# yuki-koyama/sequential-line-search

Hardware: AMD Instinct MI355X
Metric: GP-fit+acq-max step time (ms) and candidate-evals/sec at N=8192 D=64 (higher is better)
Workload: dtype f64

## Files before the change

### sequential-line-search_amd/csrc/capi.hip

```cpp
#include <cstddef>
#include <cstring>
#include <algorithm>
#include <cmath>
#include <cstdlib>
#include <cstring>
#include <atomic>
#include <map>
#include <memory>
#include <condition_variable>
#include <mutex>
#include <shared_mutex>

#include "common.hpp"
#include "kernels.hpp"
#include "lbfgs_driver.hpp"

using namespace slsk;


namespace slsk {
static thread_local char g_err[512] = "";
void set_error(const char* fmt, ...) {
    va_list ap;
    va_start(ap, fmt);
// ... 322 lines not shown
    if (launches) *launches = it == ctx->prof.end() ? 0 : it->second.launches;
    return SLS_OK;
}

static void h2d(sls_ctx* c, double* dst, const double* src, size_t n) {
    SLS_HIP(hipMemcpyAsync(dst, src, n * sizeof(double), hipMemcpyHostToDevice, c->stream));
}
static void d2h(sls_ctx* c, double* dst, const double* src, size_t n) {
    SLS_HIP(hipMemcpyAsync(dst, src, n * sizeof(double), hipMemcpyDeviceToHost, c->stream));
}
static void sync(sls_ctx* c) { SLS_HIP(hipStreamSynchronize(c->stream)); }
static const size_t IO_STAGE_MAX = (size_t)4 << 20;

static void check_theta(const double* theta, int D) {
    SLS_REQUIRE(theta != nullptr, "theta is NULL");
    SLS_REQUIRE(theta[0] > 0.0, "theta[0] (signal variance) must be positive");
    for (int d = 0; d < D; ++d) SLS_REQUIRE(theta[1 + d] > 0.0, "length scale %d must be positive", d);
}

static void d2h_matrix(sls_ctx* c, double* dst, const double* src, int N, int Np) {
    SLS_HIP(hipMemcpy2DAsync(dst, (size_t)N * 8, src, (size_t)Np * 8, (size_t)N * 8, N, hipMemcpyDeviceToHost, c->stream));
}
static void h2d_matrix(sls_ctx* c, double* dst, const double* src, int N, int Np) {
    SLS_HIP(hipMemcpy2DAsync(dst, (size_t)Np * 8, src, (size_t)N * 8, (size_t)N * 8, N, hipMemcpyHostToDevice, c->stream));
}

struct sls_gp {
    sls_ctx* ctx = nullptr;
    int D = 0, N = 0, Np = 0, Dp = 0, Dcols = 0, kernel = 0;
    double a = 0, b = 0;
    std::vector<double> theta, Xh, yh;
    std::vector<double> il_h, ypad_h;
    bool host_stale = false;
    DBuf X, y, inv_ell, XT, XaT, nx, L, Linv, Kinv, U, alpha, tvec, mu_data, scal, gemv_part, idx_buf;
    const double* linv_clean_p = nullptr;
    int linv_clean_np = 0;
    long* d_idx = nullptr;
    HostBuf sum;
    int best_index = 0;
    double mu_best = 0, logdet = 0;
    DBuf Ks, Cs, P, Vs, parts, Gs, Gm, Gpart, XsT, ns, raw, outv;
    int ws_chunk = 0;
    DBuf pair_mu, pair_sg, pair_dmu, pair_dsg;
    LbfgsWs lb;
    DBuf eubo_Ks, eubo_Cs, eubo_XsT, eubo_ns, eubo_parts, eubo_Gs, eubo_Gm, eubo_Kd;
    int eubo_chunk = 0, eubo_np = 0;
    HostBuf eubo_best;
    int sigma_mode = 0;
    long generation = 0;
    long stat_issued = 0, stat_cap = 0;
    int stat_rounds = 0, stat_live_end = 0;
    HostBuf zc;
    HostBuf io;
    double* io_stage(size_t doubles) {
        if (io.host && doubles * 8 > io.bytes) (void)hipStreamSynchronize(ctx->stream);
        io.ensure(ctx, doubles * 8, false);
        return io.host;
    }
    std::shared_mutex state_mtx;
};

static bool gp_fit_small_ok(const sls_gp* g) {
    if (g->N > NLL_SMALL_MAX_N || g->Np != 128 || g->D > 128) return false;
    return tune_on(TUNE_FIT_SMALL);
}

static std::atomic<long> g_gp_generation{0};
static void gp_fit_device(sls_gp* g) {
    g->generation = ++g_gp_generation;
    sls_ctx* c = g->ctx;
    const int N = g->N, Np = g->Np, D = g->D;
    if (gp_fit_small_ok(g)) {
        GpFitSmallArgs f;
        f.X = g->X.p; f.y = g->y.p; f.inv_ell = g->inv_ell.p;
        f.D = D; f.N = N; f.Dcols = g->Dcols; f.a = g->a; f.b = g->b;
        f.XT = g->XT.p; f.nx = g->nx.p; f.XaT = g->XaT.p; f.L = g->L.p; f.Linv = g->Linv.p; f.U = g->U.p; f.Kinv = g->Kinv.p;
        f.alpha = g->alpha.p; f.mu_data = g->mu_data.p; f.scal = g->scal.p; f.d_idx = g->d_idx; f.info = c->d_info;
        f.summary = g->sum.dev;
        f.x_lds = tune_on(TUNE_SMALL_XLDS) ? 1 : 0;
        SLS_HIP(hipMemsetAsync(c->d_info, 0, 64, c->stream));
        ProfScope ps(c, "fit_small");
        launch_gp_fit_small(c->stream, g->kernel, f);
        return;
    }
    KernelSpec ks{g->kernel, g->a};
    {
        ProfScope ps(c, "gram");
        launch_prep_points(c->stream, g->X.p, D, N, g->inv_ell.p, g->XT.p, Np, Np, g->Dcols, g->nx.p);
        launch_gram_sym(c->stream, g->XT.p, Np, g->Dp, g->nx.p, Np, N, ks, g->b, g->L.p, true);
    }
    SLS_HIP(hipMemsetAsync(c->d_info, 0, 64, c->stream));
    if (g->linv_clean_p != g->Linv.p || g->linv_clean_np != Np) {
        launch_fill(c->stream, g->Linv.p, (long)Np * Np, 0.0);
        g->linv_clean_p = g->Linv.p;
        g->linv_clean_np = Np;
    }
    c->potrf_tick_rearm();
    int* df_sync = c->potrf_df_sync(Np);
    if (potri_fused_applies(Np, df_sync != nullptr)) {
        ProfScope ps(c, "potri");
        if (!launch_potri(c->stream, g->L.p, Np, g->Linv.p, g->U.p, g->Kinv.p, c->d_info, df_sync))
            ps.rename("potrf+trtri+lauum");
    } else {
        {
            ProfScope ps(c, "potrf");
            launch_potrf(c->stream, g->L.p, Np, g->Linv.p, c->d_info, 0, df_sync);
        }
        {
            ProfScope ps(c, "trtri");
            launch_trtri(c->stream, g->L.p, Np, g->Linv.p, g->Kinv.p, g->U.p);
        }
        {
            ProfScope ps(c, "lauum");
            launch_lauum(c->stream, g->U.p, Np, g->Kinv.p);
        }
    }
    launch_gemv_n(c->stream, g->Linv.p, Np, g->y.p, g->tvec.p, g->gemv_part.p, true);
    launch_gemv_t(c->stream, g->Linv.p, Np, g->tvec.p, g->alpha.p, true);
    launch_scale_rows(c->stream, g->XT.p, g->alpha.p, g->XaT.p, Np, Np, g->Dcols);
    if (g->sigma_mode == 1) launch_transpose_full(c->stream, g->Linv.p, g->U.p, Np);
    launch_fit_summary(c->stream, g->y.p, g->alpha.p, g->b, N, g->mu_data.p, g->L.p, Np, c->d_info, g->scal.p, g->d_idx, g->sum.dev);
}

static void gp_fetch_summary(sls_gp* g, int attempt = 0) {
    sls_ctx* c = g->ctx;
    sync(c);
    const double* sm = g->sum.host;
    const int info[2] = {(int)sm[3], (int)sm[4]};
    if (potrf_gave_up(c, info[1], attempt)) {
        gp_fit_device(g);
        gp_fetch_summary(g, 1);
        return;
    }
    if (info[0] != 0) {
        set_error("Cholesky failed: K_y is not positive definite (pivot %d)", info[0] - 1);
        throw HipFail{SLS_ERR_NOT_SPD};
    }
    g->best_index = (int)sm[2];
    g->mu_best = sm[0];
    g->logdet = sm[1];
}
static void gp_setup(sls_gp* g) {
    sls_ctx* ctx = g->ctx;
    const int D = g->D, N = (int)g->yh.size();
    g->N = N;
    g->Np = round_up(N, 128); g->Dp = round_up(D, 16); g->Dcols = round_up(D, 128);
    const size_t Np = g->Np;
    g->X.ensure((size_t)D * N); g->y.ensure(Np); g->inv_ell.ensure(g->Dcols);
    g->XT.ensure(Np * g->Dcols); g->XaT.ensure(Np * g->Dcols); g->nx.ensure(Np);
    g->L.ensure(Np * Np); g->Linv.ensure(Np * Np); g->Kinv.ensure(Np * Np); g->U.ensure(Np * Np);
    g->alpha.ensure(Np); g->tvec.ensure(Np); g->mu_data.ensure(Np); g->scal.ensure(8);
    g->gemv_part.ensure((Np / 128) * Np);
    g->ws_chunk = 0;
    g->idx_buf.ensure(8);
    g->d_idx = reinterpret_cast<long*>(g->idx_buf.p);
    g->sum.ensure(ctx, (size_t)(16 + D) * 8, true);
    g->il_h.assign(g->Dcols, 0.0);
    g->ypad_h.assign(Np, 0.0);
    for (int d = 0; d < D; ++d) g->il_h[d] = 1.0 / g->theta[1 + d];
    std::copy(g->yh.begin(), g->yh.end(), g->ypad_h.begin());
    h2d(ctx, g->X.p, g->Xh.data(), (size_t)D * N);
    h2d(ctx, g->y.p, g->ypad_h.data(), Np);
    h2d(ctx, g->inv_ell.p, g->il_h.data(), g->Dcols);
    gp_fit_device(g);
    gp_fetch_summary(g);
}

extern "C" int sls_gp_create(sls_ctx* ctx, const double* X, int D, int N, const double* y, const double* theta, double b,
                             int kernel, sls_gp** out) {
    SLS_TRY
    CtxCall call_(ctx);
    SLS_REQUIRE(ctx && out, "sls_gp_create: NULL argument");
    SLS_REQUIRE(D >= 1 && N >= 1, "sls_gp_create: need D >= 1 and N >= 1 (got D=%d N=%d)", D, N);
    SLS_REQUIRE(X && y, "sls_gp_create: X / y is NULL");
    SLS_REQUIRE(kernel == SLS_KERNEL_ARD_SQUARED_EXPONENTIAL || kernel == SLS_KERNEL_ARD_MATERN52, "unknown kernel %d", kernel);
    SLS_REQUIRE(b >= 0.0, "noise level must be >= 0");
    check_theta(theta, D);
    SLS_HIP(hipSetDevice(ctx->device));
    std::unique_ptr<sls_gp> g(new sls_gp());
    g->ctx = ctx; g->D = D; g->kernel = kernel; g->a = theta[0]; g->b = b;
    g->theta.assign(theta, theta + D + 1);
    g->Xh.assign(X, X + (size_t)D * N);
// ... 192 lines not shown
            ProfScope ps(c, "cross_gram");
            if (point_major) launch_prep_points(c->stream, xr + (size_t)s0 * D, D, sc, g->inv_ell.p, g->XsT.p, ldk, Sp, g->Dcols, g->ns.p);
            else launch_prep_cands(c->stream, xr + s0, ldr, D, sc, g->inv_ell.p, g->XsT.p, ldk, Sp, g->Dcols, g->ns.p);
            launch_cross_gram(c->stream, g->XsT.p, ldk, g->ns.p, Sp, g->XT.p, Np, g->nx.p, Np, N, g->Dp, ks, g->alpha.p, g->Ks.p, Cs,
                              ldk, mu_part, ca_part);
        }
        int split_first = 0x7fffffff;
        const bool solve_grad = g->sigma_mode == 1 && (want_grad || !tri_predict());
        {
            ProfScope ps(c, want_grad ? "acq_gemm" : "var_gemm");
            if (solve_grad) {
                g->Vs.ensure((size_t)chunk_max * Np);
                launch_gemm_plain(c->stream, g->Ks.p, ldk, false, g->Linv.p, Np, false, g->Vs.p, ldk, Sp / 128, Np / 128, Np, 1.0, 0.0);
                split_first = launch_acq_gemm(c->stream, g->Vs.p, Cs, ldk, Sp, g->U.p, Np, g->P.p, kw_part, cw_part, c->d_info + 32);
            } else if (want_grad || !tri_predict())
                split_first = launch_acq_gemm(c->stream, g->Ks.p, Cs, ldk, Sp, g->Kinv.p, Np, g->P.p, kw_part, cw_part, c->d_info + 32);
            else
                launch_var_gemm(c->stream, g->Ks.p, ldk, Sp, g->Linv.p, Np, kw_part, cw_part);
        }
        double* kw_solve = nullptr;
        if (solve_grad) {
            kw_solve = cw_part + (size_t)2 * nbt * ldk;
            ProfScope ps(c, "var_gemm");
            launch_var_gemm(c->stream, g->Ks.p, ldk, Sp, g->Linv.p, Np, kw_solve, kw_solve + (size_t)2 * nbt * ldk);
        }
        if (want_grad) {
            ProfScope ps(c, "grad_gemm");
            double* part = nullptr;
            if (D <= 64 && grad_gemm_wants_split(Sp)) {
                g->Gpart.ensure((size_t)8 * Sp * 64);
                part = g->Gpart.p;
            }
            launch_grad_gemm(c->stream, g->P.p, Cs, ldk, Sp, g->XT.p, g->XaT.p, Np, Np, D <= 64 ? -g->Dcols : g->Dcols, g->Gs.p, g->Gm.p,
                             part);
        }
        {
            ProfScope ps(c, "finalize");
            FinalizeArgs f;
            f.S = sc; f.D = D; f.nbt = nbt; f.ldk = ldk; f.ntm = Sp / 128; f.split_first = split_first;
            f.mu_part = mu_part; f.ca_part = ca_part; f.kw_part = kw_part; f.cw_part = cw_part;
            f.kw_solve_part = kw_solve;
            f.Gs = g->Gs.p; f.Gm = g->Gm.p; f.XsT = g->XsT.p; f.inv_ell = g->inv_ell.p;
            f.a = g->a; f.mu_best = g->mu_best; f.ucb_h = o.ucb_h; f.acq = o.acq;
            f.ldo = o.ldo;
            f.mu = o.mu ? o.mu + s0 : nullptr;
            f.sigma = o.sigma ? o.sigma + s0 : nullptr;
            f.dmu = o.dmu ? o.dmu + s0 : nullptr;
            f.dsigma = o.dsigma ? o.dsigma + s0 : nullptr;
            f.val = o.val ? o.val + s0 : nullptr;
            f.grad = o.grad ? o.grad + s0 : nullptr;
            launch_finalize(c->stream, f);
        }
    }
}

constexpr int WAVE_PATH_MAX_POINTS = 4096;
static bool wave_path_dims(const sls_gp* g) { return tune_on(TUNE_WAVE_PATH) && g->D <= WAVE_PATH_MAX_D; }
static bool wave_path_applies(const sls_gp* g, int count) {
    return wave_path_dims(g) && g->Np <= WAVE_PATH_MAX_NP && count <= WAVE_PATH_MAX_POINTS;
}
static void wave_model_args(const sls_gp* g, WaveArgs& w) {
    w.D = g->D; w.N = g->N; w.Np = g->Np;
    w.matern = g->kernel == SLS_KERNEL_ARD_MATERN52;
    w.a = g->a; w.mu_best = g->mu_best;
    w.XT = g->XT.p; w.inv_ell = g->inv_ell.p; w.Kinv = g->Kinv.p; w.alpha = g->alpha.p;
    w.solve_sigma = g->sigma_mode == 1; w.Linv = g->Linv.p; w.U = g->U.p;
    w.useful = nullptr;
// ... 578 lines not shown
        }
        double* kw_solve = solve ? cw_part[0] + (size_t)2 * nbt * ldk : nullptr;
        for (int o = 0; o < 2; ++o) {
            ProfScope ps(c, "cross_gram");
            launch_prep_cands(c->stream, xr + (size_t)o * D * ldr + s0, ldr, D, sc, g->inv_ell.p, XsT[o], ldk, Sp, g->Dcols, ns[o]);
            launch_cross_gram(c->stream, XsT[o], ldk, ns[o], Sp, g->XT.p, Np, g->nx.p, Np, N, g->Dp, ks, g->alpha.p, Ks[o], Cs[o], ldk,
                              mu_part[o], ca_part[o]);
        }
        {
            ProfScope ps(c, "eubo");
            launch_pair_diff(c->stream, Ks[0], Ks[1], ldk, Np, g->eubo_Kd.p);
        }
        if (solve) {
            {
                ProfScope ps(c, "acq_gemm");
                launch_gemm_plain(c->stream, g->eubo_Kd.p, ldk, false, g->Linv.p, Np, false, g->Vs.p, ldk, Sp / 128, Np / 128, Np, 1.0, 0.0);
            }
            ProfScope ps(c, "var_gemm");
            launch_var_gemm(c->stream, g->eubo_Kd.p, ldk, Sp, g->Linv.p, Np, kw_solve, kw_solve + (size_t)2 * nbt * ldk);
        }
        int split_first = 0x7fffffff;
        for (int o = 0; o < 2; ++o) {
            {
                ProfScope ps(c, "acq_gemm");
                split_first = launch_acq_gemm(c->stream, solve ? g->Vs.p : g->eubo_Kd.p, Cs[o], ldk, Sp, solve ? g->U.p : g->Kinv.p, Np,
                                              g->P.p, kw_part[o], cw_part[o], c->d_info + 32);
            }
            ProfScope ps(c, "grad_gemm");
            double* part = nullptr;
            if (D <= 64 && grad_gemm_wants_split(Sp)) {
                g->Gpart.ensure((size_t)8 * Sp * 64);
                part = g->Gpart.p;
            }
            launch_grad_gemm(c->stream, g->P.p, Cs[o], ldk, Sp, g->XT.p, g->XaT.p, Np, Np, D <= 64 ? -g->Dcols : g->Dcols, Gs[o], Gm[o], part);
        }
        {
            ProfScope ps(c, "eubo");
            EuboFinalizeArgs f;
            f.S = sc; f.D = D; f.nbt = nbt; f.ntm = Sp / 128; f.split_first = split_first; f.kernel = g->kernel; f.ldk = ldk;
            for (int o = 0; o < 2; ++o) {
                f.mu_part[o] = mu_part[o]; f.ca_part[o] = ca_part[o]; f.cw_part[o] = cw_part[o];
                f.Gs[o] = Gs[o]; f.Gm[o] = Gm[o]; f.XsT[o] = XsT[o];
            }
            f.kw_part = kw_part[0]; f.kw_solve_part = kw_solve; f.inv_ell = g->inv_ell.p; f.a = g->a;
            f.ldo = ldo;
            f.val = val ? val + s0 : nullptr;
            f.grad = grad ? grad + s0 : nullptr;
            launch_eubo_finalize(c->stream, f);
        }
    }
}

extern "C" int sls_eubo_eval(sls_gp* g, const double* pairs, int M, double* val, double* grad) {
    SLS_TRY
    CtxCall call_(g);
    SLS_REQUIRE(g != nullptr, "sls_eubo_eval: gp is NULL");
    SLS_REQUIRE(pairs != nullptr, "sls_eubo_eval: pairs is NULL");
    SLS_REQUIRE(M >= 0, "sls_eubo_eval: M = %d", M);
    if (M == 0) return SLS_OK;
    std::shared_lock<std::shared_mutex> state_(g->state_mtx);
    sls_ctx* c = g->ctx;
    const int Mp = round_up(M, 128), D2 = 2 * g->D;
    std::vector<double> t((size_t)Mp * D2, 0.5);
    for (int m = 0; m < M; ++m)
        for (int r = 0; r < D2; ++r) t[(size_t)m + (size_t)r * Mp] = pairs[r + (size_t)m * D2];
    g->raw.ensure((size_t)Mp * D2);
    h2d(c, g->raw.p, t.data(), (size_t)Mp * D2);
// ... 201 lines not shown
    }
    g->Xh.insert(g->Xh.end(), x, x + D);
    g->yh.push_back(y_new);
    if (N % 128 == 0) {
        gp_setup(g);
        return SLS_OK;
    }
    upload_candidates(g, x, 1, g->raw, 128);
    ensure_eval_ws(g, 128);
    g->outv.ensure(4 * (size_t)Np + 8);
    double* kvec = g->outv.p;
    double* uvec = kvec + Np;
    double* lvec = uvec + Np;
    double* tmp = lvec + Np;
    double* scal = tmp + Np;
    KernelSpec ks{g->kernel, g->a};
    launch_prep_cands(c->stream, g->raw.p, 128, D, 1, g->inv_ell.p, g->XsT.p, 128, 128, g->Dcols, g->ns.p);
    double* Cs = (g->kernel == SLS_KERNEL_ARD_MATERN52) ? g->Cs.p : g->Ks.p;
    launch_cross_gram(c->stream, g->XsT.p, 128, g->ns.p, 128, g->XT.p, Np, g->nx.p, Np, N, g->Dp, ks, nullptr, g->Ks.p, Cs, 128,
                      nullptr, nullptr);
    SLS_HIP(hipMemcpy2DAsync(kvec, 8, g->Ks.p, 128 * 8, 8, Np, hipMemcpyDeviceToDevice, c->stream));
    launch_gemv_n(c->stream, g->Kinv.p, Np, kvec, uvec, g->gemv_part.p);
    launch_gemv_n(c->stream, g->Linv.p, Np, kvec, lvec, g->gemv_part.p, true);
    launch_append_dots(c->stream, kvec, uvec, lvec, g->y.p, N, scal);
    const double kappa = g->a + g->b;
    launch_append_update(c->stream, g->Kinv.p, g->L.p, g->Linv.p, g->alpha.p, Np, N, uvec, lvec, scal, kappa, y_new);
    SLS_HIP(hipMemcpyAsync(g->y.p + N, &g->yh[N], 8, hipMemcpyHostToDevice, c->stream));
    g->X.ensure((size_t)D * (N + 1));
    SLS_HIP(hipMemcpyAsync(g->X.p, g->Xh.data(), (size_t)D * (N + 1) * 8, hipMemcpyHostToDevice, c->stream));
    g->N = N + 1;
    g->generation = ++g_gp_generation;
    launch_prep_points(c->stream, g->X.p, D, N + 1, g->inv_ell.p, g->XT.p, Np, Np, g->Dcols, g->nx.p);
    launch_scale_rows(c->stream, g->XT.p, g->alpha.p, g->XaT.p, Np, Np, g->Dcols);
    if (g->sigma_mode == 1) launch_transpose_full(c->stream, g->Linv.p, g->U.p, Np);
    SLS_HIP(hipMemsetAsync(c->d_info, 0, 64, c->stream));
    launch_fit_summary(c->stream, g->y.p, g->alpha.p, g->b, N + 1, g->mu_data.p, g->L.p, Np, c->d_info, g->scal.p, g->d_idx, g->sum.dev);
    gp_fetch_summary(g);
    SLS_REQUIRE(std::isfinite(g->logdet), "sls_gp_append_point: the extended K_y is not positive definite");
    SLS_CATCH
}
```

### sequential-line-search_amd/csrc/gemm_f64.hpp

```cpp
#pragma once
#include <hip/hip_runtime.h>

namespace slsk {

typedef double d4_t __attribute__((ext_vector_type(4)));
typedef double d2_t __attribute__((ext_vector_type(2)));

constexpr int GEMM_BM = 128;
constexpr int GEMM_BN = 128;
constexpr int GEMM_BK = 16;
constexpr int GEMM_THREADS = 256;
constexpr int GEMM_LDS_MC_LD = 144;
constexpr int GEMM_LDS_KC_LD = 18;
constexpr int GEMM_LDS_TILE = 16 * 144;
constexpr int GEMM_LDS_BYTES = 4 * GEMM_LDS_TILE * 8;

struct Acc {
    d4_t v[4][4];
    __device__ __forceinline__ void zero() {
#pragma unroll
        for (int i = 0; i < 4; ++i)
#pragma unroll
            for (int j = 0; j < 4; ++j) v[i][j] = d4_t{0.0, 0.0, 0.0, 0.0};
    }
// ... 280 lines not shown
        if (more) {
            if (DIRECT_A) issue_a(k0 + GEMM_BK, cur ^ BUF);
            else stage_load<A_KC>(sa, A, lda, k0 + GEMM_BK, tid);
            load_b(k0 + GEMM_BK);
        }
        const double* la = lds + cur;
        const double* lb = lds + cur + A_SLAB;
#pragma unroll
        for (int kk = 0; kk < 4; ++kk) {
            double af[2], bf[4];
#pragma unroll
            for (int i = 0; i < 2; ++i)
                af[i] = A_KC ? frag_read<true>(la, wm + 16 * i, kk, lane)
                             : la[(4 * kk + (lane >> 4)) * A_LD + wm + 16 * i + (lane & 15)];
#pragma unroll
            for (int j = 0; j < 4; ++j) bf[j] = frag_read<true>(lb, 16 * j, kk, lane);
#pragma unroll
            for (int i = 0; i < 2; ++i)
#pragma unroll
                for (int j = 0; j < 4; ++j)
                    acc.v[i][j] = __builtin_amdgcn_mfma_f64_16x16x4f64(bf[j], af[i], acc.v[i][j], 0, 0, 0);
        }
        const int nxt = cur ^ BUF;
        if (more) {
            if (!DIRECT_A) stage_store<A_KC>(sa, lds + nxt, tid);
            store_b(lds + nxt + A_SLAB);
        }
        if (DIRECT_A) asm volatile("s_waitcnt vmcnt(0)" ::: "memory");
        __syncthreads();
        cur = nxt;
    }
}

__device__ __forceinline__ int acc_m(int i) {
    const int lane = threadIdx.x & 63, wave = threadIdx.x >> 6;
    return (wave & 1) * 64 + 16 * i + (lane & 15);
}
__device__ __forceinline__ int acc_n(int j, int r) {
    const int lane = threadIdx.x & 63, wave = threadIdx.x >> 6;
    return (wave >> 1) * 64 + 16 * j + (lane >> 4) + 4 * r;
}

template <bool HEAVY = false, class F>
__device__ __forceinline__ void acc_tile_by_columns(const Acc& acc, double* lds, F&& f) {
    const int lane = threadIdx.x & 63, wave = __builtin_amdgcn_readfirstlane(threadIdx.x >> 6);
#pragma unroll
    for (int half = 0; half < 2; ++half) {
        __syncthreads();
        if ((wave >> 1) == half) {
#pragma unroll
            for (int i = 0; i < 4; ++i)
#pragma unroll
                for (int j = 0; j < 4; ++j)
#pragma unroll
                    for (int r = 0; r < 4; ++r)
                        lds[(16 * j + (lane >> 4) + 4 * r) * GEMM_LDS_MC_LD + (wave & 1) * 64 + 16 * i + (lane & 15)] = acc.v[i][j][r];
        }
        __syncthreads();
        if constexpr (HEAVY) {
#pragma unroll 2
            for (int q = 0; q < 16; ++q) {
                const int c = wave + 4 * q;
                const d2_t v = *reinterpret_cast<const d2_t*>(lds + c * GEMM_LDS_MC_LD + 2 * lane);
                f(64 * half + c, 2 * lane, v);
            }
        } else {
// ... 19 lines not shown
```

### sequential-line-search_amd/csrc/kernels.hpp

```cpp
#pragma once
#include <cstdlib>
#include <hip/hip_runtime.h>

#include "tuning.hpp"
#include "../../include/sls_hip.h"

#include <mutex>
#include <map>
#include <set>
#include <utility>

namespace slsk {

inline void ensure_dyn_lds(const void* fn, int bytes) {
    static std::mutex mtx;
    static std::map<std::pair<int, const void*>, int> done;
    int dev = 0;
    (void)hipGetDevice(&dev);
    std::lock_guard<std::mutex> lock(mtx);
    int& have = done[{dev, fn}];
    if (bytes > have) {
        if (hipFuncSetAttribute(fn, hipFuncAttributeMaxDynamicSharedMemorySize, bytes) != hipSuccess) (void)hipGetLastError();
        have = bytes;
    }
// ... 89 lines not shown
struct MapOptArgs {
    const double* X;
    const double* XTr;
    double* kc;
    int x_lds = 1;
    int D, N, ny, nh, log_hyper, noiseless;
    const double* y_fixed;
    double a0, b0, r0;
    double mu_a, mu_b, mu_r, s2_a, s2_b, s2_r;
    double btl_scale;
    int n_prefs, flat_len;
    const int *pref_off, *pref_flat;
    const int *csc_off, *csc_ent;
    double* btl_scratch;
    const double *z0, *lower, *upper;
    int max_evals;
    double ftol_rel, xtol_rel;
    int budget;
    int eval_only;
    int fresh;
    double* state;
    double* out;
    int* info;
    long long* trace;
};
void launch_map_opt(hipStream_t s, int kernel, const MapOptArgs& args);

int launch_acq_gemm(hipStream_t s, const double* Ks, const double* Cs, long ldk, int Sp, const double* Kinv, int Np, double* P,
                    double* kw_part, double* cw_part, int* sync = nullptr);
void launch_var_gemm(hipStream_t s, const double* Ks, long ldk, int Sp, const double* Linv, int Np, double* kw_part,
                     double* cw_part);
inline bool grad_gemm_wants_split(int Sp) { return !tune_set(TUNE_GRAD_SPLIT_TILES) || 2 * (Sp / 128) < tune(TUNE_GRAD_SPLIT_TILES, 0); }
void launch_grad_gemm(hipStream_t s, const double* P, const double* Cs, long ldk, int Sp, const double* XT, const double* XaT,
                      long ld, int Np, int Dcols, double* Gs, double* Gm, double* part = nullptr, int passes = 2);
struct FinalizeArgs {
    int S, D, nbt;
    int ntm, split_first;
    long ldk;
    const double *mu_part, *ca_part, *kw_part, *cw_part, *Gs, *Gm, *XsT, *inv_ell;
    const double* kw_solve_part = nullptr;
    double a, mu_best, ucb_h;
    int acq;
    long ldo;
    double *mu, *sigma, *dmu, *dsigma, *val, *grad;
};
void launch_finalize(hipStream_t s, const FinalizeArgs& a);

void launch_combine(hipStream_t s, int S, int D, long ld, const double* mu, const double* sigma, const double* dmu,
                    const double* dsigma, int acq, double mu_best, double ucb_h, double* val, double* grad);

void launch_mes_combine(hipStream_t s, int S, int D, long ld, const double* mu, const double* sigma, const double* dmu,
                        const double* dsigma, const double* y_star, int K, double* val, double* grad);
void launch_mes_terms(hipStream_t s, const double* t, long n, double* g, double* dg);

void launch_logei_combine(hipStream_t s, int S, int D, long ld, const double* mu, const double* sigma, const double* dmu,
                          const double* dsigma, double mu_best, double* val, double* grad);
void launch_logei_terms(hipStream_t s, const double* u, long n, double* log_h, double* b1, double* b2);

void launch_pair_diff(hipStream_t s, const double* Ka, const double* Kb, long ldk, int Np, double* Kd);
struct EuboFinalizeArgs {
    int S, D, nbt;
    int ntm, split_first;
    int kernel;
    long ldk;
    const double *mu_part[2], *ca_part[2], *cw_part[2], *Gs[2], *Gm[2], *XsT[2];
    const double *kw_part, *inv_ell;
    const double* kw_solve_part = nullptr;
// ... 141 lines not shown
```

### sequential-line-search_amd/csrc/kernels_acq.hip

```cpp
#include <cstdlib>

#include "gemm_f64.hpp"
#include "kernels.hpp"
#include "../../include/sls_hip.h"

namespace slsk {

template <bool MATERN, bool HALF>
__device__ __forceinline__ void acq_tile(int t, int nhalf, int ntm, int ntn, const double* __restrict__ Ks, const double* __restrict__ Cs,
                                         long ldk, const double* __restrict__ Kinv, int Np, double* __restrict__ P,
                                         double* __restrict__ kw_part, double* __restrict__ cw_part, double* lds) {
    const int GM = 8;
    const int gsz = GM * ntn;
    const int g = t / gsz, w = t % gsz;
    const int gm = min(GM, ntm - g * GM);
    const int tm = g * GM + (w % gm), tn = w / gm;
    const int m0 = tm * GEMM_BM, n0 = tn * GEMM_BN;
    Acc acc;
    acc.zero();
    gemm_tile<false, false, HALF ? 2 : 4, true>(acc, Ks + m0, ldk, Kinv + n0, (long)Np, 0, Np, lds, nhalf);
    const int lane = threadIdx.x & 63, wave = threadIdx.x >> 6;
    constexpr int NJ = HALF ? 2 : 4;
    const int nbase = HALF ? 64 * nhalf + (wave >> 1) * 32 : (wave >> 1) * 64;
    double* red = lds;
// ... 238 lines not shown
                     double* cw_part) {
    ensure_dyn_lds((const void*)var_gemm_kernel, GEMM_LDS_BYTES);
    const int ntm = Sp / GEMM_BM, ntn = Np / GEMM_BN;
    const int pair = (ntm * ntn < 1024 && ntn > 1) ? 1 : 0;
    const int grid = pair ? ntm * ((ntn + 1) / 2) : ntm * ntn;
    hipLaunchKernelGGL(var_gemm_kernel, dim3(grid), dim3(GEMM_THREADS), GEMM_LDS_BYTES, s, Ks, ldk, Sp, Linv, Np, kw_part, cw_part,
                       pair);
}

__global__ __launch_bounds__(256, 2) void grad_gemm_kernel(const double* __restrict__ P, const double* __restrict__ Cs, long ldk,
                                                           int Sp, const double* __restrict__ XT, const double* __restrict__ XaT,
                                                           long ld, int Np, int Dcols, double* __restrict__ Gs,
                                                           double* __restrict__ Gm) {
    extern __shared__ __attribute__((aligned(16))) char smem[];
    double* lds = reinterpret_cast<double*>(smem);
    const int ntm = Sp / GEMM_BM;
    const int tm = blockIdx.x % ntm, tn = blockIdx.x / ntm;
    const int m0 = tm * GEMM_BM, n0 = tn * GEMM_BN;
    const double* A = blockIdx.y == 0 ? P : Cs;
    const double* B = blockIdx.y == 0 ? XT : XaT;
    double* C = blockIdx.y == 0 ? Gs : Gm;
    Acc acc;
    acc.zero();
    gemm_tile<false, true>(acc, A + m0, ldk, B + (long)n0 * ld, ld, 0, Np, lds);
#pragma unroll
    for (int i = 0; i < 4; ++i)
#pragma unroll
        for (int j = 0; j < 4; ++j)
#pragma unroll
            for (int r = 0; r < 4; ++r) C[(long)(m0 + acc_m(i)) + (long)(n0 + acc_n(j, r)) * ldk] = acc.v[i][j][r];
}

constexpr int GRAD64_A_LD = 136;
__global__ __launch_bounds__(256, 3) void grad_gemm64_kernel(const double* __restrict__ P, const double* __restrict__ Cs, long ldk,
                                                             int Sp, const double* __restrict__ XT, const double* __restrict__ XaT,
                                                             long ld, int Np, double* __restrict__ Gs, double* __restrict__ Gm,
                                                             double* __restrict__ part) {
    extern __shared__ __attribute__((aligned(16))) char smem[];
    double* lds = reinterpret_cast<double*>(smem);
    const int m0 = blockIdx.x * GEMM_BM;
    const double* A = blockIdx.y == 0 ? P : Cs;
    const double* B = blockIdx.y == 0 ? XT : XaT;
    const bool split = gridDim.z > 1;
    double* C = split ? part + ((long)blockIdx.z * 2 + blockIdx.y) * (long)Sp * 64 : (blockIdx.y == 0 ? Gs : Gm);
    const long ldc = split ? (long)Sp : ldk;
    const int q = Np / 4;
    Acc64 tot;
    tot.zero();
    const int c0 = split ? blockIdx.z : 0, c1 = split ? blockIdx.z + 1 : 4;
    for (int c = c0; c < c1; ++c) {
        Acc64 acc;
        acc.zero();
        gemm_tile_n64<false, GRAD64_A_LD>(acc, A + m0, ldk, B, ld, c * q, (c + 1) * q, lds);
#pragma unroll
        for (int i = 0; i < 2; ++i)
#pragma unroll
            for (int j = 0; j < 4; ++j) tot.v[i][j] = (c == c0) ? acc.v[i][j] : tot.v[i][j] + acc.v[i][j];
    }
    const int lane = threadIdx.x & 63, wm = (threadIdx.x >> 6) * 32;
#pragma unroll
    for (int i = 0; i < 2; ++i)
#pragma unroll
        for (int j = 0; j < 4; ++j)
#pragma unroll
            for (int r = 0; r < 4; ++r)
                C[(long)(m0 + wm + 16 * i + (lane & 15)) + (long)(16 * j + (lane >> 4) + 4 * r) * ldc] = tot.v[i][j][r];
}

__global__ __launch_bounds__(256) void grad_reduce4_kernel(const double* __restrict__ part, int Sp, long ldk, double* __restrict__ Gs,
                                                           double* __restrict__ Gm, int passes) {
    const long idx = blockIdx.x * 256L + threadIdx.x;
    if (idx >= (long)Sp * 64) return;
    const long n = idx % Sp, d = idx / Sp;
    const long stride = (long)Sp * 64;
    for (int y = 0; y < passes; ++y) {
        const double* p = part + (long)y * stride + idx;
        const double v = ((p[0] + p[2 * stride]) + p[4 * stride]) + p[6 * stride];
        (y == 0 ? Gs : Gm)[n + d * ldk] = v;
    }
}

void launch_grad_gemm(hipStream_t s, const double* P, const double* Cs, long ldk, int Sp, const double* XT, const double* XaT,
                      long ld, int Np, int Dcols, double* Gs, double* Gm, double* part, int passes) {
    ensure_dyn_lds((const void*)grad_gemm_kernel, GEMM_LDS_BYTES);
    ensure_dyn_lds((const void*)grad_gemm64_kernel, gemm_n64_lds_bytes<GRAD64_A_LD>());
    if (Dcols < 0) {
        const bool split = part != nullptr && grad_gemm_wants_split(Sp);
        hipLaunchKernelGGL(grad_gemm64_kernel, dim3(Sp / GEMM_BM, passes, split ? 4 : 1), dim3(GEMM_THREADS), gemm_n64_lds_bytes<GRAD64_A_LD>(), s, P, Cs,
                           ldk, Sp, XT, XaT, ld, Np, Gs, Gm, part);
        if (split)
            hipLaunchKernelGGL(grad_reduce4_kernel, dim3((unsigned)(((long)Sp * 64 + 255) / 256)), dim3(256), 0, s, part, Sp, ldk, Gs, Gm,
                               passes);
        return;
    }
    const int nt = (Sp / GEMM_BM) * (Dcols / GEMM_BN);
    hipLaunchKernelGGL(grad_gemm_kernel, dim3(nt, passes), dim3(GEMM_THREADS), GEMM_LDS_BYTES, s, P, Cs, ldk, Sp, XT, XaT, ld, Np, Dcols,
                       Gs, Gm);
}

__global__ __launch_bounds__(256) void finalize_kernel(FinalizeArgs p) {
    const int n = blockIdx.x * 256 + threadIdx.x;
    if (n >= p.S) return;
    double mu = 0.0, ca = 0.0, kw = 0.0, cw = 0.0;
    const int tm_ = n >> 7, grp_ = tm_ >> 3;
    const int gm_ = min(8, p.ntm - 8 * grp_);
    const int tile_base = grp_ * 8 * p.nbt + (tm_ - 8 * grp_);
    #pragma unroll 8
    for (int t = 0; t < p.nbt; ++t) {
        mu += p.mu_part[(long)t * p.ldk + n];
        ca += p.ca_part[(long)t * p.ldk + n];
        double kt = p.kw_part[(long)(2 * t) * p.ldk + n], ct = p.cw_part[(long)(2 * t) * p.ldk + n];
        if (tile_base + t * gm_ >= p.split_first) {
            kt += p.kw_part[(long)(2 * t + 1) * p.ldk + n];
            ct += p.cw_part[(long)(2 * t + 1) * p.ldk + n];
        }
        kw += kt;
        cw += ct;
    }
    if (p.kw_solve_part) {
        kw = 0.0;
        for (int t = 0; t < p.nbt; ++t) kw += p.kw_solve_part[(long)(2 * t) * p.ldk + n];
    }
// ... 709 lines not shown
```

### sequential-line-search_amd/csrc/kernels_gram.hip

```cpp
#include "gemm_f64.hpp"
#include "kernels.hpp"
#include "../../include/sls_hip.h"

namespace slsk {

constexpr int PREP_PTS = 64, PREP_DCH = 64, PREP_LD = PREP_DCH + 1;
template <bool CAND_MAJOR>
__global__ __launch_bounds__(256) void prep_kernel(const double* __restrict__ X, long ldr, int D, int M,
                                                   const double* __restrict__ inv_ell, double* __restrict__ XT, long ld, int Mp,
                                                   int Dcols, double* __restrict__ norms) {
    __shared__ double vs[PREP_PTS * PREP_LD];
    __shared__ double ils[PREP_DCH];
    const int i0 = blockIdx.x * PREP_PTS, tid = threadIdx.x;
    const int p = tid & 63, w = tid >> 6, i = i0 + p;
    double s = 0.0;
    for (int d0 = 0; d0 < Dcols; d0 += PREP_DCH) {
        if (tid < PREP_DCH) ils[tid] = d0 + tid < D ? inv_ell[d0 + tid] : 0.0;
        double raw[PREP_DCH / 4];
        if (CAND_MAJOR) {
#pragma unroll
            for (int k = 0; k < PREP_DCH / 4; ++k) {
                const int d = d0 + w + 4 * k;
                raw[k] = (i < M && d < D) ? X[i + (long)d * ldr] : 0.5;
            }
// ... 32 lines not shown
            for (int dd = 0; dd < dn; ++dd) {
                const double v = vs[tid * PREP_LD + dd];
                s += v * v;
            }
        }
        __syncthreads();
    }
    if (tid < PREP_PTS && i0 + tid < Mp) norms[i0 + tid] = s;
}

void launch_prep_points(hipStream_t s, const double* X, int D, int M, const double* inv_ell, double* XT, long ld, int Mp,
                        int Dcols, double* norms) {
    hipLaunchKernelGGL(prep_kernel<false>, dim3((Mp + PREP_PTS - 1) / PREP_PTS), dim3(256), 0, s, X, 0L, D, M, inv_ell, XT, ld, Mp, Dcols,
                       norms);
}
void launch_prep_cands(hipStream_t s, const double* xr, long ldr, int D, int M, const double* inv_ell, double* XT, long ld,
                       int Mp, int Dcols, double* norms) {
    hipLaunchKernelGGL(prep_kernel<true>, dim3((Mp + PREP_PTS - 1) / PREP_PTS), dim3(256), 0, s, xr, ldr, D, M, inv_ell, XT, ld, Mp, Dcols,
                       norms);
}

__global__ __launch_bounds__(256) void scale_rows_kernel(const double* __restrict__ XT, const double* __restrict__ alpha,
                                                         double* __restrict__ XaT, long ld, int Np, int Dcols) {
    const int i = blockIdx.x * 256 + threadIdx.x;
    if (i >= Np) return;
    const double al = alpha[i];
    const int d0 = blockIdx.y * 16;
    double v[16];
#pragma unroll
    for (int k = 0; k < 16; ++k) v[k] = XT[i + (long)(d0 + k) * ld];
#pragma unroll
    for (int k = 0; k < 16; ++k) XaT[i + (long)(d0 + k) * ld] = al * v[k];
}
void launch_scale_rows(hipStream_t s, const double* XT, const double* alpha, double* XaT, long ld, int Np, int Dcols) {
    hipLaunchKernelGGL(scale_rows_kernel, dim3((Np + 255) / 256, Dcols / 16), dim3(256), 0, s, XT, alpha, XaT, ld, Np, Dcols);
}

__global__ __launch_bounds__(256, 2) void gram_sym_kernel(const double* __restrict__ XT, long ld, int Dp,
                                                          const double* __restrict__ nx, int Np, int N, int kernel, double a,
                                                          double b, double* __restrict__ K, int lower_only) {
    extern __shared__ __attribute__((aligned(16))) char smem[];
    double* lds = reinterpret_cast<double*>(smem);
    const int nt = Np / GEMM_BM;
    int tm, tn;
    if (lower_only) {
        const int t = xcd_remap(blockIdx.x, nt * (nt + 1) / 2);
        tm = (int)((sqrt(8.0 * t + 1.0) - 1.0) * 0.5);
        while (tm * (tm + 1) / 2 > t) --tm;
        while ((tm + 1) * (tm + 2) / 2 <= t) ++tm;
        tn = t - tm * (tm + 1) / 2;
    } else {
        const int t = xcd_remap(blockIdx.x, nt * nt);
        tm = t % nt;
        tn = t / nt;
    }
    const int m0 = tm * GEMM_BM, n0 = tn * GEMM_BN;
    Acc acc;
    acc.zero();
    gemm_tile<false, false>(acc, XT + m0, ld, XT + n0, ld, 0, Dp, lds);
    acc_tile_by_columns<true>(acc, lds, [&](int col, int row, d2_t dot) {
        const int gj = n0 + col;
        const double nj = nx[gj];
        const d2_t ni = *reinterpret_cast<const d2_t*>(nx + m0 + row);
        d2_t out;
#pragma unroll
        for (int e = 0; e < 2; ++e) {
// ... 90 lines not shown
```

### sequential-line-search_amd/csrc/tuning.hpp

```cpp
#pragma once
#include <atomic>
#include <cstdlib>
#include <mutex>

namespace slsk {
#define SLS_TUNING_KEYS(X)                                                                                                      \
    X(POOL_MB) X(FIT_SMALL) X(TRI_PREDICT) X(WAVE_PATH) X(IO_STAGE) X(EVAL_ZEROCOPY) X(WAVE_TRACE) X(COMPACT) \
    X(NLL_SMALL) X(SMALL_ZEROCOPY) X(NLL_BATCH) X(MAP_DEVICE) X(MAP_TRACE) X(SMALL_XLDS) X(MULTI_RCCL) X(PERSIST)                \
    X(ACQ_WG_PER_CU) X(GATE_PHASE) X(TAIL_SPLIT) X(LBFGS_REG) X(TRI_WG_PER_CU) X(POTRF_MODE) X(POTRF_DNBO) X(POTRF_NBO)          \
    X(LAUUM_N64) X(TRTRI_NARROW) X(POTRI_FUSED) X(POTRF_STREAM) X(POTRF_SPLIT) X(POTRI_W1) X(POTRF_TIMEOUT_TICKS) X(POTRF_DNEAR) X(POTRI_PLAST)  \
    X(POTRI_CX) X(POTRI_CK) X(WAVE_STAGE) X(WAVE_COOP) X(GRAD_SPLIT_TILES) X(EVAL_SLOTS) X(GATE_EVERY) X(POTRF_FUSE_SYRK) X(POTRI_POOL) X(POTRF_POOL) X(POTRI_POOL_KEEP) X(POTRI_POOL_NEAR) X(POTRI_POOL_NEAR_W)
enum TuneKey {
#define SLS_TK(name) TUNE_##name,
    SLS_TUNING_KEYS(SLS_TK)
#undef SLS_TK
    TUNE_COUNT
};
struct SlsTuning {
    std::atomic<long long> word[TUNE_COUNT];
};
namespace tuning_detail {
inline SlsTuning& table() {
    static SlsTuning t;
    return t;
}
inline void parse() {
    static const char* const names[TUNE_COUNT] = {
#define SLS_TK(name) "SLS_" #name,
        SLS_TUNING_KEYS(SLS_TK)
#undef SLS_TK
    };
    SlsTuning& t = table();
    for (int k = 0; k < TUNE_COUNT; ++k) {
        const char* v = getenv(names[k]);
        t.word[k].store(v ? (((long long)atol(v)) << 1) | 1 : 0, std::memory_order_relaxed);
    }
}
}
inline const SlsTuning& tuning() {
    static std::once_flag once;
    std::call_once(once, tuning_detail::parse);
    return tuning_detail::table();
}
inline void tuning_reload() {
// ... 12 lines not shown
```

Measured before the change: 537,900.

## Add point-major copies of XT/XaT and direct-slab B loads in grad GEMM

After each fit, a new kernel writes point-major (N×64) copies of the scaled and unscaled design matrices. The D≤64 gradient GEMM gains a variant, on by default via GRAD_B_DIRECT, that streams B rows from these contiguous copies straight into LDS using the same slab-load path as A. The aim is to replace strided column-major B gathers in the hot acquisition-gradient kernel with contiguous loads. It costs an extra transpose kernel per fit or update and two extra Np×64 buffers.

```diff
diff --git a/sequential-line-search_amd/csrc/capi.hip b/sequential-line-search_amd/csrc/capi.hip
--- a/sequential-line-search_amd/csrc/capi.hip
+++ b/sequential-line-search_amd/csrc/capi.hip
@@ -378,6 +378,7 @@
     std::vector<double> theta, Xh, yh;
     std::vector<double> il_h, ypad_h;
     bool host_stale = false;
+    DBuf XdT, XadT;
     DBuf X, y, inv_ell, XT, XaT, nx, L, Linv, Kinv, U, alpha, tvec, mu_data, scal, gemv_part, idx_buf;
     const double* linv_clean_p = nullptr;
     int linv_clean_np = 0;
@@ -411,6 +412,13 @@
     return tune_on(TUNE_FIT_SMALL);
 }
 
+static void gp_point_major(sls_gp* g) {
+    if (g->D > 64) return;
+    launch_point_major(g->ctx->stream, g->XT.p, g->XaT.p, g->Np, g->Np, g->Dcols, g->XdT.p, g->XadT.p);
+}
+static const double* gp_xdt(const sls_gp* g) { return g->D <= 64 ? g->XdT.p : nullptr; }
+static const double* gp_xadt(const sls_gp* g) { return g->D <= 64 ? g->XadT.p : nullptr; }
+
 static std::atomic<long> g_gp_generation{0};
 static void gp_fit_device(sls_gp* g) {
     g->generation = ++g_gp_generation;
@@ -427,6 +435,7 @@
         SLS_HIP(hipMemsetAsync(c->d_info, 0, 64, c->stream));
         ProfScope ps(c, "fit_small");
         launch_gp_fit_small(c->stream, g->kernel, f);
+        gp_point_major(g);
         return;
     }
     KernelSpec ks{g->kernel, g->a};
@@ -464,6 +473,7 @@
     launch_gemv_n(c->stream, g->Linv.p, Np, g->y.p, g->tvec.p, g->gemv_part.p, true);
     launch_gemv_t(c->stream, g->Linv.p, Np, g->tvec.p, g->alpha.p, true);
     launch_scale_rows(c->stream, g->XT.p, g->alpha.p, g->XaT.p, Np, Np, g->Dcols);
+    gp_point_major(g);
     if (g->sigma_mode == 1) launch_transpose_full(c->stream, g->Linv.p, g->U.p, Np);
     launch_fit_summary(c->stream, g->y.p, g->alpha.p, g->b, N, g->mu_data.p, g->L.p, Np, c->d_info, g->scal.p, g->d_idx, g->sum.dev);
 }
@@ -494,6 +504,7 @@
     const size_t Np = g->Np;
     g->X.ensure((size_t)D * N); g->y.ensure(Np); g->inv_ell.ensure(g->Dcols);
     g->XT.ensure(Np * g->Dcols); g->XaT.ensure(Np * g->Dcols); g->nx.ensure(Np);
+    if (D <= 64) { g->XdT.ensure(Np * 64); g->XadT.ensure(Np * 64); }
     g->L.ensure(Np * Np); g->Linv.ensure(Np * Np); g->Kinv.ensure(Np * Np); g->U.ensure(Np * Np);
     g->alpha.ensure(Np); g->tvec.ensure(Np); g->mu_data.ensure(Np); g->scal.ensure(8);
     g->gemv_part.ensure((Np / 128) * Np);
@@ -752,7 +763,7 @@
                 part = g->Gpart.p;
             }
             launch_grad_gemm(c->stream, g->P.p, Cs, ldk, Sp, g->XT.p, g->XaT.p, Np, Np, D <= 64 ? -g->Dcols : g->Dcols, g->Gs.p, g->Gm.p,
-                             part);
+                             part, 2, gp_xdt(g), gp_xadt(g));
         }
         {
             ProfScope ps(c, "finalize");
@@ -1397,7 +1408,8 @@
                 g->Gpart.ensure((size_t)8 * Sp * 64);
                 part = g->Gpart.p;
             }
-            launch_grad_gemm(c->stream, g->P.p, Cs[o], ldk, Sp, g->XT.p, g->XaT.p, Np, Np, D <= 64 ? -g->Dcols : g->Dcols, Gs[o], Gm[o], part);
+            launch_grad_gemm(c->stream, g->P.p, Cs[o], ldk, Sp, g->XT.p, g->XaT.p, Np, Np, D <= 64 ? -g->Dcols : g->Dcols, Gs[o], Gm[o], part, 2,
+                             gp_xdt(g), gp_xadt(g));
         }
         {
             ProfScope ps(c, "eubo");
@@ -1665,6 +1677,7 @@
     g->generation = ++g_gp_generation;
     launch_prep_points(c->stream, g->X.p, D, N + 1, g->inv_ell.p, g->XT.p, Np, Np, g->Dcols, g->nx.p);
     launch_scale_rows(c->stream, g->XT.p, g->alpha.p, g->XaT.p, Np, Np, g->Dcols);
+    gp_point_major(g);
     if (g->sigma_mode == 1) launch_transpose_full(c->stream, g->Linv.p, g->U.p, Np);
     SLS_HIP(hipMemsetAsync(c->d_info, 0, 64, c->stream));
     launch_fit_summary(c->stream, g->y.p, g->alpha.p, g->b, N + 1, g->mu_data.p, g->L.p, Np, c->d_info, g->scal.p, g->d_idx, g->sum.dev);
diff --git a/sequential-line-search_amd/csrc/gemm_f64.hpp b/sequential-line-search_amd/csrc/gemm_f64.hpp
--- a/sequential-line-search_amd/csrc/gemm_f64.hpp
+++ b/sequential-line-search_amd/csrc/gemm_f64.hpp
@@ -336,6 +336,72 @@
     }
 }
 
+constexpr int GEMM_N64_LDS_BD = 16 * 64;
+template <int A_LD>
+constexpr int gemm_n64_bd_lds_bytes() {
+    return 2 * (16 * A_LD + GEMM_N64_LDS_BD) * 8;
+}
+template <int A_LD>
+__device__ __forceinline__ void gemm_tile_n64_bd(Acc64& acc, const double* __restrict__ A, long lda, const double* __restrict__ Bd, int kb,
+                                                 int ke, double* lds) {
+    constexpr int A_SLAB = 16 * A_LD;
+    constexpr int BUF = A_SLAB + GEMM_N64_LDS_BD;
+    if (kb >= ke) return;
+    const int tid = threadIdx.x, lane = tid & 63;
+    const int wave = __builtin_amdgcn_readfirstlane(tid >> 6);
+    const int wm = wave * 32;
+    const unsigned lds_base = (unsigned)(unsigned long long)(__attribute__((address_space(3))) double*)lds;
+    const unsigned a_off = 16u * lane;
+    const unsigned b_off = 8u * (unsigned)((lane >> 5) * 64 + 2 * ((lane & 31) ^ ((lane >> 5) * 8)));
+    auto issue = [&](int k0, int bufoff) {
+        const double* Arow = A + (long)(k0 + 4 * wave) * lda;
+        const double* Brow = Bd + (long)(k0 + 4 * wave) * 64;
+#pragma unroll
+        for (int r = 0; r < 4; ++r)
+            slab_row_to_lds_saddr(Arow + (long)r * lda, a_off, lds_base + 8u * (unsigned)(bufoff + (4 * wave + r) * A_LD));
+#pragma unroll
+        for (int q = 0; q < 2; ++q)
+            slab_row_to_lds_saddr(Brow + 128 * q, b_off, lds_base + 8u * (unsigned)(bufoff + A_SLAB + (2 * wave + q) * 128));
+    };
+    const int x = lane & 15, g = lane >> 4, odd = g & 1;
+    const int bp0 = (g >> 1) * 128 + odd * 64 + x + 16 * odd;
+    const int bp1 = (g >> 1) * 128 + odd * 64 + x + 16 - 16 * odd;
+    int ap[2][4];
+#pragma unroll
+    for (int b = 0; b < 2; ++b)
+#pragma unroll
+        for (int kk = 0; kk < 4; ++kk) {
+            ap[b][kk] = b * BUF + 4 * kk * A_LD + g * A_LD + wm + x;
+            asm volatile("" : "+v"(ap[b][kk]));
+        }
+    auto compute = [&](int bufoff) {
+        const double* lb = lds + bufoff + A_SLAB;
+#pragma unroll
+        for (int kk = 0; kk < 4; ++kk) {
+            double af[2], bf[4];
+#pragma unroll
+            for (int i = 0; i < 2; ++i) af[i] = lds[ap[bufoff ? 1 : 0][kk] + 16 * i];
+#pragma unroll
+            for (int j = 0; j < 4; ++j) bf[j] = lb[2 * kk * 128 + ((j & 1) ? bp1 : bp0) + 32 * (j >> 1)];
+#pragma unroll
+            for (int i = 0; i < 2; ++i)
+#pragma unroll
+                for (int j = 0; j < 4; ++j)
+                    acc.v[i][j] = __builtin_amdgcn_mfma_f64_16x16x4f64(bf[j], af[i], acc.v[i][j], 0, 0, 0);
+        }
+    };
+    issue(kb, 0);
+    ring_wait_barrier<0>();
+    for (int k0 = kb; k0 < ke; k0 += 2 * GEMM_BK) {
+        issue(k0 + GEMM_BK, BUF);
+        compute(0);
+        ring_wait_barrier<0>();
+        issue(k0 + 2 * GEMM_BK < ke ? k0 + 2 * GEMM_BK : kb, 0);
+        compute(BUF);
+        ring_wait_barrier<0>();
+    }
+}
+
 __device__ __forceinline__ int acc_m(int i) {
     const int lane = threadIdx.x & 63, wave = threadIdx.x >> 6;
     return (wave & 1) * 64 + 16 * i + (lane & 15);
diff --git a/sequential-line-search_amd/csrc/kernels.hpp b/sequential-line-search_amd/csrc/kernels.hpp
--- a/sequential-line-search_amd/csrc/kernels.hpp
+++ b/sequential-line-search_amd/csrc/kernels.hpp
@@ -145,7 +145,9 @@
                      double* cw_part);
 inline bool grad_gemm_wants_split(int Sp) { return !tune_set(TUNE_GRAD_SPLIT_TILES) || 2 * (Sp / 128) < tune(TUNE_GRAD_SPLIT_TILES, 0); }
 void launch_grad_gemm(hipStream_t s, const double* P, const double* Cs, long ldk, int Sp, const double* XT, const double* XaT,
-                      long ld, int Np, int Dcols, double* Gs, double* Gm, double* part = nullptr, int passes = 2);
+                      long ld, int Np, int Dcols, double* Gs, double* Gm, double* part = nullptr, int passes = 2,
+                      const double* XdT = nullptr, const double* XadT = nullptr);
+void launch_point_major(hipStream_t s, const double* XT, const double* XaT, long ld, int Np, int Dcols, double* XdT, double* XadT);
 struct FinalizeArgs {
     int S, D, nbt;
     int ntm, split_first;
diff --git a/sequential-line-search_amd/csrc/kernels_acq.hip b/sequential-line-search_amd/csrc/kernels_acq.hip
--- a/sequential-line-search_amd/csrc/kernels_acq.hip
+++ b/sequential-line-search_amd/csrc/kernels_acq.hip
@@ -294,6 +294,7 @@
 }
 
 constexpr int GRAD64_A_LD = 136;
+template <bool BD>
 __global__ __launch_bounds__(256, 3) void grad_gemm64_kernel(const double* __restrict__ P, const double* __restrict__ Cs, long ldk,
                                                              int Sp, const double* __restrict__ XT, const double* __restrict__ XaT,
                                                              long ld, int Np, double* __restrict__ Gs, double* __restrict__ Gm,
@@ -313,7 +314,8 @@
     for (int c = c0; c < c1; ++c) {
         Acc64 acc;
         acc.zero();
-        gemm_tile_n64<false, GRAD64_A_LD>(acc, A + m0, ldk, B, ld, c * q, (c + 1) * q, lds);
+        if constexpr (BD) gemm_tile_n64_bd<GRAD64_A_LD>(acc, A + m0, ldk, B, c * q, (c + 1) * q, lds);
+        else gemm_tile_n64<false, GRAD64_A_LD>(acc, A + m0, ldk, B, ld, c * q, (c + 1) * q, lds);
 #pragma unroll
         for (int i = 0; i < 2; ++i)
 #pragma unroll
@@ -343,13 +345,18 @@
 }
 
 void launch_grad_gemm(hipStream_t s, const double* P, const double* Cs, long ldk, int Sp, const double* XT, const double* XaT,
-                      long ld, int Np, int Dcols, double* Gs, double* Gm, double* part, int passes) {
+                      long ld, int Np, int Dcols, double* Gs, double* Gm, double* part, int passes, const double* XdT,
+                      const double* XadT) {
     ensure_dyn_lds((const void*)grad_gemm_kernel, GEMM_LDS_BYTES);
-    ensure_dyn_lds((const void*)grad_gemm64_kernel, gemm_n64_lds_bytes<GRAD64_A_LD>());
     if (Dcols < 0) {
+        const bool bd = XdT != nullptr && tune_on(TUNE_GRAD_B_DIRECT);
+        const auto kern = bd ? grad_gemm64_kernel<true> : grad_gemm64_kernel<false>;
+        const int lds_bytes = gemm_n64_lds_bytes<GRAD64_A_LD>();
+        static_assert(gemm_n64_bd_lds_bytes<GRAD64_A_LD>() <= gemm_n64_lds_bytes<GRAD64_A_LD>(), "one LDS size for both forms");
+        ensure_dyn_lds((const void*)kern, lds_bytes);
         const bool split = part != nullptr && grad_gemm_wants_split(Sp);
-        hipLaunchKernelGGL(grad_gemm64_kernel, dim3(Sp / GEMM_BM, passes, split ? 4 : 1), dim3(GEMM_THREADS), gemm_n64_lds_bytes<GRAD64_A_LD>(), s, P, Cs,
-                           ldk, Sp, XT, XaT, ld, Np, Gs, Gm, part);
+        hipLaunchKernelGGL(kern, dim3(Sp / GEMM_BM, passes, split ? 4 : 1), dim3(GEMM_THREADS), lds_bytes, s, P, Cs, ldk, Sp,
+                           bd ? XdT : XT, bd ? XadT : XaT, ld, Np, Gs, Gm, part);
         if (split)
             hipLaunchKernelGGL(grad_reduce4_kernel, dim3((unsigned)(((long)Sp * 64 + 255) / 256)), dim3(256), 0, s, part, Sp, ldk, Gs, Gm,
                                passes);
diff --git a/sequential-line-search_amd/csrc/kernels_gram.hip b/sequential-line-search_amd/csrc/kernels_gram.hip
--- a/sequential-line-search_amd/csrc/kernels_gram.hip
+++ b/sequential-line-search_amd/csrc/kernels_gram.hip
@@ -88,6 +88,19 @@
 #pragma unroll
     for (int k = 0; k < 16; ++k) XaT[i + (long)(d0 + k) * ld] = al * v[k];
 }
+__global__ __launch_bounds__(256) void point_major_kernel(const double* __restrict__ XT, const double* __restrict__ XaT, long ld, int Np,
+                                                          int Dcols, double* __restrict__ XdT, double* __restrict__ XadT) {
+    const int i = blockIdx.x * 256 + threadIdx.x;
+    if (i >= Np) return;
+    const int d0 = blockIdx.y * 16;
+    const double* src = blockIdx.z == 0 ? XT : XaT;
+    double* dst = blockIdx.z == 0 ? XdT : XadT;
+    for (int k = 0; k < 16; ++k) dst[(long)i * 64 + d0 + k] = (d0 + k < Dcols) ? src[i + (long)(d0 + k) * ld] : 0.0;
+}
+void launch_point_major(hipStream_t s, const double* XT, const double* XaT, long ld, int Np, int Dcols, double* XdT, double* XadT) {
+    hipLaunchKernelGGL(point_major_kernel, dim3((Np + 255) / 256, 4, 2), dim3(256), 0, s, XT, XaT, ld, Np, Dcols, XdT, XadT);
+}
+
 void launch_scale_rows(hipStream_t s, const double* XT, const double* alpha, double* XaT, long ld, int Np, int Dcols) {
     hipLaunchKernelGGL(scale_rows_kernel, dim3((Np + 255) / 256, Dcols / 16), dim3(256), 0, s, XT, alpha, XaT, ld, Np, Dcols);
 }
diff --git a/sequential-line-search_amd/csrc/tuning.hpp b/sequential-line-search_amd/csrc/tuning.hpp
--- a/sequential-line-search_amd/csrc/tuning.hpp
+++ b/sequential-line-search_amd/csrc/tuning.hpp
@@ -9,7 +9,7 @@
     X(NLL_SMALL) X(SMALL_ZEROCOPY) X(NLL_BATCH) X(MAP_DEVICE) X(MAP_TRACE) X(SMALL_XLDS) X(MULTI_RCCL) X(PERSIST)                \
     X(ACQ_WG_PER_CU) X(GATE_PHASE) X(TAIL_SPLIT) X(LBFGS_REG) X(TRI_WG_PER_CU) X(POTRF_MODE) X(POTRF_DNBO) X(POTRF_NBO)          \
     X(LAUUM_N64) X(TRTRI_NARROW) X(POTRI_FUSED) X(POTRF_STREAM) X(POTRF_SPLIT) X(POTRI_W1) X(POTRF_TIMEOUT_TICKS) X(POTRF_DNEAR) X(POTRI_PLAST)  \
-    X(POTRI_CX) X(POTRI_CK) X(WAVE_STAGE) X(WAVE_COOP) X(GRAD_SPLIT_TILES) X(EVAL_SLOTS) X(GATE_EVERY) X(POTRF_FUSE_SYRK) X(POTRI_POOL) X(POTRF_POOL) X(POTRI_POOL_KEEP) X(POTRI_POOL_NEAR) X(POTRI_POOL_NEAR_W)
+    X(POTRI_CX) X(POTRI_CK) X(WAVE_STAGE) X(WAVE_COOP) X(GRAD_SPLIT_TILES) X(EVAL_SLOTS) X(GATE_EVERY) X(POTRF_FUSE_SYRK) X(POTRI_POOL) X(POTRF_POOL) X(POTRI_POOL_KEEP) X(POTRI_POOL_NEAR) X(POTRI_POOL_NEAR_W) X(GRAD_B_DIRECT)
 enum TuneKey {
 #define SLS_TK(name) TUNE_##name,
     SLS_TUNING_KEYS(SLS_TK)
```

New measurement: 538,300, median of 6. About the same (+0.1%).
